# antoinedesbois/Ray-Tracer-Rust

Hardware: AMD Instinct MI355X
Metric: Mrays/sec + frame ms, big_bunny.obj @ 1920x1080 (higher is better)
Workload: dtype f32

## Files before the change

### ray-tracer-rust_amd/csrc/rtx_api.cpp

```cpp
#include <hip/hip_runtime.h>

#include <algorithm>
#include <chrono>
#include <cmath>
#include <cstddef>
#include <cstdio>
#include <cstdlib>
#include <cstring>
#include <initializer_list>
#include <map>
#include <memory>
#include <mutex>
#include <new>
#include <vector>

#include "../../include/rtx.h"
#include "rtx_aim.h"
#include "rtx_device.h"
#include "rtx_light.h"
#include "rtx_query.h"
#include "rtx_shade.h"
#include "rtx_view.h"
#include "scene_prep.h"

// ... 67 lines not shown
    template <class T>
    T *as() const { return static_cast<T *>(static_cast<void *>(mem_)); }
private:
    Owned<void *, Free> mem_;
    size_t cap_ = 0;
};
using DeviceBuffer = GrowOnly<alloc_device, hipFree>;
using PinnedBuffer = GrowOnly<alloc_pinned, hipHostFree>;

struct Sized { DeviceBuffer &buffer; size_t bytes; };
int reserve_all(std::initializer_list<Sized> list)
{
    for (const Sized &s : list) {
        const int rc = s.buffer.reserve(s.bytes);
        if (rc != RTX_OK) return rc;
    }
    return RTX_OK;
}

class DeviceState {
public:
    explicit DeviceState(int dev) : device(dev) {}
    const int device;
    bool uploaded = false;
    size_t last_tiles = 0;
    unsigned long long launches = 0;
    Stream stream;
    Event ev0, ev1;
    Event ring[RTX_TIMING_RING][3];
    Event q_sorted;
    DeviceBuffer nodes, primary_nodes, ref_nodes, tris, shade, samples, lights, light_tour, thr, planes, light_boxes;
    DeviceBuffer d_out, d_counters;
    DeviceBuffer d_redo;
    PinnedBuffer h_stage;
    struct { DeviceBuffer hits, pix_slot, tiles, chunks, results, acc, ctr, buckets, cut; } ws;
    DeviceBuffer q_first, q_second, q_out;
    struct { DeviceBuffer keys, keys_sorted, index, index_sorted, temp; } q_sort;
    struct {
        DeviceBuffer nodes, links;
        float eye[3] = {0.0f, 0.0f, 0.0f};
        hipStream_t on = nullptr;
        bool valid = false;
    } aimed;
    struct {
        DeviceBuffer points;
        Event used;
    } lit;
private:
    ~DeviceState() = default;
    friend struct ReleaseOnDevice;
};

struct ReleaseOnDevice {
    void operator()(DeviceState *st) const
    {
        DeviceGuard g(st->device);
        if (g.status() != hipSuccess) return;
        if (st->stream) (void)hipStreamSynchronize(st->stream);
        delete st;
    }
};

struct DeviceSlot {
    std::mutex mu;
    std::unique_ptr<DeviceState, ReleaseOnDevice> st;
};
// ... 190 lines not shown
uint32_t tiles_rows(uint32_t height, uint32_t first_tile, uint32_t tile_stride, uint32_t tile_rows)
{
    if (!tile_rows || !tile_stride) return 0;
    uint64_t rows = 0;
    for (uint64_t t = first_tile; t * tile_rows < height; t += tile_stride) {
        const uint64_t r0 = t * tile_rows;
        rows += (height - r0 < tile_rows) ? (height - r0) : tile_rows;
    }
    return static_cast<uint32_t>(rows);
}

void fill_stats(RtxStats *s, uint64_t primary_rays, uint32_t shadow_rays_per_hit, const unsigned long long *c,
                double kernel_ms, double total_ms)
{
    std::memset(s, 0, sizeof *s);
    s->primary_rays = primary_rays;
    s->primary_hits = c[0];
    s->shadow_rays = c[0] * shadow_rays_per_hit;
    s->rays = s->primary_rays + s->shadow_rays;
    s->box_tests = c[1];
    s->tri_tests = c[2];
    s->wave_node_visits = c[3];
    s->wave_tri_visits = c[4];
    s->redo_tiles = c[5];
    s->kernel_ms = kernel_ms;
    s->total_ms = total_ms;
}

template <class Before>
int render_launch(DeviceState &st, const rtx::DeviceScene &S, const rtx::TileSpec &ts, uint8_t *d_out,
                  unsigned long long *d_counters, unsigned long long *d_wave_prof, hipStream_t stream, Before before)
{
    int rc;
    if ((rc = st.d_redo.reserve(rtx::trace_redo_bytes(S, ts))) != RTX_OK) return rc;
    rtx::StreamWorkspace ws{};
    bool use_ws = false;
    if (!d_wave_prof && (rc = reserve_stream_ws(st, S, ts, &ws, &use_ws)) != RTX_OK) return rc;
    if ((rc = before()) != RTX_OK) return rc;
    const Event *slot = st.ring[st.launches % RTX_TIMING_RING];
    hipEvent_t phases[3] = {slot[0], slot[1], slot[2]};
    RTX_HIP(rtx::launch_trace_shade(S, ts, d_out, st.d_redo.as<uint32_t>(), use_ws ? &ws : nullptr, d_counters, d_wave_prof,
                                    kernel_variant(), stream, d_wave_prof ? nullptr : phases));
    if (!d_wave_prof && ts.local_rows) ++st.launches;
    return RTX_OK;
}

int launch_on(RtxScene *scene, DeviceSlot &slot, const rtx::TileSpec &ts, bool count)
{
    int rc = ensure_uploaded(scene, slot);
    if (rc != RTX_OK) return rc;
    DeviceState &st = *slot.st;
    const size_t bytes = static_cast<size_t>(ts.local_rows) * scene->prep.width * 3u;
    if ((rc = st.d_out.reserve(bytes ? bytes : 16)) != RTX_OK) return rc;
    unsigned long long *counters = count ? st.d_counters.as<unsigned long long>() : nullptr;
    rc = render_launch(st, device_scene(scene, st), ts, st.d_out.as<uint8_t>(), counters, nullptr, st.stream, [&]() -> int {
        if (count) RTX_HIP(hipMemsetAsync(counters, 0, rtx::kNumCounters * sizeof(unsigned long long), st.stream));
        RTX_HIP(hipEventRecord(st.ev0, st.stream));
        return RTX_OK;
    });
    if (rc != RTX_OK) return rc;
    RTX_HIP(hipEventRecord(st.ev1, st.stream));
    return RTX_OK;
}


rtxq::KeyBox query_key_box(const rtx::PreparedScene &p)
{
    rtxq::KeyBox box{};
    if (p.nodes.empty()) return box;
    const rtx::NodeRec &root = p.nodes[(p.n_global != 0u && p.nodes.size() > 2u) ? 2u : 0u];
    for (int a = 0; a < 3; ++a) {
        const float extent = root.bmax[a] - root.bmin[a];
        const float scale = static_cast<float>(1u << rtxq::kMortonBitsPerAxis) / extent;
        box.lo[a] = root.bmin[a];
        box.scale[a] = (extent > 0.0f && scale > 0.0f && scale < 0x1p100f) ? scale : 0.0f;
// ... 950 lines not shown
```

### ray-tracer-rust_amd/csrc/rtx_device.h

```cpp
#pragma once

#include <hip/hip_runtime.h>

#include <cstdint>

#include "scene_prep.h"

namespace rtx {

struct DeviceScene {
    const NodeRec  *nodes;
    const NodeRec  *primary_nodes;
    const float    *light_tour;
    const NodeRec  *ref_nodes;
    const TriRec   *tris;
    const ShadeRec *shade;
    const TriRec   *planes;
    const float2   *samples;
    const float    *light_points;
    const float    *gamma_thr;
    const float    *light_boxes;
    uint32_t n_nodes, n_ref_nodes, n_samples, n_wide;
    uint32_t width, height;
    uint32_t nb_ray, nb_light;
// ... 46 lines not shown
    uint32_t *buckets;
    CutEntry *cut;
};
constexpr uint32_t kCutInnerFlag = 1u << 29, kCutEndMask = (1u << 26) - 1u;
constexpr uint32_t kCutStreamRecords = kMaxCut + 1u;
__host__ __device__ inline size_t cut_stream_offset(size_t tiles)
{
    return (tiles * kMaxCut * sizeof(CutEntry) + 63u) & ~static_cast<size_t>(63u);
}
struct StreamWorkspaceBytes { size_t hits, pix_slot, tiles, chunks, results, acc, ctr, buckets, cut; };
static_assert(kMaxCut >= 1u && kMaxCut <= 51u && kCutWords * kMaxCut <= 512u, "RTX_MAX_CUT: 1 .. 51 (one staged word per work-item of 512)");
constexpr uint32_t kTileCutShift = 8u;
constexpr uint32_t kTileCompactHits = 8u;
constexpr uint32_t kTileChunk0Kept = 4u;
StreamWorkspaceBytes stream_workspace_bytes(const DeviceScene &S, const TileSpec &ts, uint32_t variant);
constexpr uint32_t kCostBuckets = 64u;
constexpr uint32_t kStreamCtrWords = 4u;

constexpr int kNumCounters = 8;

#ifndef RTX_LIGHT_TOUR
#define RTX_LIGHT_TOUR 1
#endif
static_assert(RTX_LIGHT_TOUR >= 0 && RTX_LIGHT_TOUR <= 2, "RTX_LIGHT_TOUR: 0, 1 or 2");

constexpr uint32_t kVariantStream = 8u;
constexpr uint32_t kVariantPacked = 16u;
constexpr uint32_t kVariantProbe = 32u;
constexpr uint32_t kVariantMask = 63u;
constexpr uint32_t kDefaultVariant = kVariantProbe | 1u;

constexpr size_t kWaveProfWords = 8;
uint32_t trace_tiles_x(const DeviceScene &S, uint32_t variant);
constexpr uint32_t kQueueRedoCount = 0u, kQueueNextTile = 1u, kQueueHeader = 4u;
size_t trace_redo_bytes(const DeviceScene &S, const TileSpec &ts);
hipError_t launch_trace_shade(const DeviceScene &S, const TileSpec &ts, uint8_t *d_out, uint32_t *d_redo,
                              const StreamWorkspace *ws, unsigned long long *d_counters,
                              unsigned long long *d_wave_prof, uint32_t variant, hipStream_t stream,
                              hipEvent_t *phase_events = nullptr);

}
```

### ray-tracer-rust_amd/csrc/rtx_kernel.hip

```cpp
#include <cstdlib>
#include "rtx_traverse.hpp"

namespace rtx {

namespace {

constexpr uint32_t kHitStride = 12u;
__device__ __forceinline__ uint32_t compact_hit_word(uint32_t record, uint32_t word)
{
    return word < 3u ? record * 3u + word : (word < 9u ? 192u + word - 3u : kNone);
}

#ifndef RTX_WAVES_PER_SIMD
#define RTX_WAVES_PER_SIMD 6
#endif
#ifndef RTX_PACKED_WAVES_PER_SIMD
#define RTX_PACKED_WAVES_PER_SIMD 4
#endif

__device__ __forceinline__ uint32_t quantise(const float *__restrict__ thr, float x)
{
    uint32_t b = 0;
#pragma unroll
    for (uint32_t step = 128; step; step >>= 1)
// ... 369 lines not shown
        }
        if (pass && leaf) {
            if (kCutEntriesUsed) out[n_out + (uint32_t)__popcll(m_leaf & below)] = CutEntry{my, my + 1u, nd};
            l_entries[n_out + (uint32_t)__popcll(m_leaf & below)] = CutEntry{my, my + 1u, nd};
            out_stream[n_out + (uint32_t)__popcll(m_leaf & below)] = nd;
            around(nd);
            w += 1u + 3u * nd.link;
        }
        n_out += n_leaf;
        if (n_exp == 0u) break;
        if (pass && !leaf) {
            const uint32_t k = (uint32_t)__popcll(m_exp & below);
            l_front[2u * k] = my + 1u;
            l_front[2u * k + 1u] = nd.info;
        }
        __builtin_amdgcn_fence(__ATOMIC_RELEASE, "wavefront");
        __builtin_amdgcn_wave_barrier();
        n_front = 2u * n_exp;
        my = l_front[lane];
        __builtin_amdgcn_fence(__ATOMIC_ACQUIRE, "wavefront");
        __builtin_amdgcn_wave_barrier();
    }
    weight = wave_sum(w);
    if (n_out >= 2u) {
        NodeDev all;
        all.lox = wave_min(ulx); all.loy = wave_min(uly); all.loz = wave_min(ulz);
        all.hix = wave_max(uhx); all.hiy = wave_max(uhy); all.hiz = wave_max(uhz);
        all.link = 0u; all.info = 0u;
        if (lane == 0) out_stream[kMaxCut] = all;
    }
    return n_out;
}

template <bool COUNT, bool FAST, bool SPHERES, bool WHOLE>
__global__ void __launch_bounds__(64 * kProbeWaves, RTX_PROBE_WAVES_PER_SIMD) probe_kernel(DeviceScene S, TileSpec ts, uint32_t tiles_x, uint32_t n_tiles,
                                                   uint32_t r, StreamWorkspace W, uint8_t *__restrict__ out,
                                                   uint32_t *__restrict__ queue, unsigned long long *__restrict__ counters)
{
    const NodeRec RTX_CONSTANT *nodes = (const NodeRec RTX_CONSTANT *)S.nodes;
    const TriRec RTX_CONSTANT *tris = (const TriRec RTX_CONSTANT *)S.tris;
    __shared__ uint32_t l_front_all[kProbeWaves][128];
    __shared__ CutEntry l_entries_all[kProbeWaves][kMaxCut];
#if RTX_ABLATION
    __shared__ __align__(16) uint32_t l_j1_block[kProbeWaves][kJ1BlockWords];
#endif
    const uint32_t lane = threadIdx.x & 63u;
    const uint32_t wave_in_group = __builtin_amdgcn_readfirstlane(threadIdx.x >> 6);
    uint32_t *const l_front = l_front_all[wave_in_group];
    static_assert(kProbeWaves == 1u, "the XCD mapping assumes one tile per workgroup");
    const uint32_t k = blockIdx.x >> 3;
    const uint32_t tile_id = ((((k >> 6) << 3) + (blockIdx.x & 7u)) << 6) + (k & 63u);
    if (tile_id >= n_tiles) return;
    uint32_t px, py, ly, tile_x, tile_y;
    tile_xy(tile_id, tiles_x, true, tile_x, tile_y);
    const bool in_frame = tile_pixel(S, ts, tile_x, tile_y, lane, px, py, ly);
    WaveCounters wc;
    float dx, dy, dz;
    primary_ray(S, in_frame, px, py, r, dx, dy, dz);
    LaneRay pr = make_ray(in_frame, S.eye[0], S.eye[1], S.eye[2], dx, dy, dz);
#if RTX_EXPERIMENT_PROBE_PHASES
    const unsigned long long pp_t0 = wall_clock64();
#endif
#if RTX_ABLATION
    const bool ok = (S.j1_mode == 2u || S.j1_mode == 3u)
        ? j1_closest_hit_blocks<COUNT>(S.j1_mode, S.tris, S.shade, S.n_prims, pr, wc, lane, l_j1_block[wave_in_group])
        : closest_hit<COUNT, FAST, SPHERES>((const NodeRec RTX_CONSTANT *)S.primary_nodes, tris, S.shade, S.n_nodes, pr, wc, S.n_global);
// ... 88 lines not shown
            (void)length_and_direction(vx, vy, vz, dist_light, sx, sy, sz);
            LaneRay sr = make_ray(hit, hx, hy, hz, sx, sy, sz);
            sr.limit = dist_light;
            WaveCounters probe;
            const bool walked = any_hit<true, FAST, SPHERES>(nodes, tris, S.shade, S.n_nodes, sr, probe, S.n_global);
            weight = (uint32_t)(probe.node_visits + probe.tri_visits);
            if (walked && n_hit == 64u && (flags & 1u)) {
                const unsigned long long occluded = ballot(sr.best_idx != kNone);
                if (lane == 0) {
                    uint32_t *kept = reinterpret_cast<uint32_t *>(W.cut + (size_t)tile_id * kMaxCut);
                    kept[0] = (uint32_t)occluded;
                    kept[1] = (uint32_t)(occluded >> 32);
                }
                flags |= kTileChunk0Kept;
            }
        }
        cost = (unsigned long long)(kChunkFixedCost + weight) * n_chunks;
        if (!(flags & 1u) && n_cut != 0u) cost *= 2u;
    }
    const bool sky = n_hit == 0u && !(flags & 2u);
    if (sky) {
        const size_t pix = (size_t)tile_id * 64u + lane;
        if (r + 1u == S.nb_ray) {
            float a0 = 0.0f, a1 = 0.0f, a2 = 0.0f;
            if (r != 0u) { a0 = W.acc[3u * pix]; a1 = W.acc[3u * pix + 1u]; a2 = W.acc[3u * pix + 2u]; }
            if (in_frame) store_pixel(S, out, px, ly, a0, a1, a2);
        } else if (r == 0u) {
            W.acc[3u * pix] = 0.0f; W.acc[3u * pix + 1u] = 0.0f; W.acc[3u * pix + 2u] = 0.0f;
        }
    }
    if (lane == 0) {
        const bool count_it = !(flags & 2u);
        const uint32_t key = (sky || (flags & 2u)) ? kNone : cost_class(cost);
#if RTX_EXPERIMENT_PROBE_PHASES
        const unsigned long long pp_t2 = wall_clock64();
        const uint32_t walk_ticks = (uint32_t)(pp_t1 - pp_t0) > 0xFFFFu ? 0xFFFFu : (uint32_t)(pp_t1 - pp_t0);
        const uint32_t rest_ticks = (uint32_t)(pp_t2 - pp_t1) > 0xFFFFu ? 0xFFFFu : (uint32_t)(pp_t2 - pp_t1);
        W.tiles[tile_id] = TileDesc{key, n_hit, flags | (n_cut << kTileCutShift), walk_ticks | (rest_ticks << 16)};
#elif RTX_EXPERIMENT_TIMELINE || RTX_EXPERIMENT_PHASES
        W.tiles[tile_id] = TileDesc{key, n_hit, flags | (n_cut << kTileCutShift), 0u};
#else
        W.tiles[tile_id] = TileDesc{key, n_hit, flags | (n_cut << kTileCutShift), counted + (count_it ? n_hit : 0u)};
#endif
        if (COUNT) {
            flush_counters<COUNT>(counters, count_it ? (unsigned long long)n_hit : 0ull, wc);
            if (counters) {
                atomicAdd(&counters[6], wc.node_visits);
                atomicAdd(&counters[7], wc.tri_visits);
            }
        }
    }
}

constexpr uint32_t kOrderHist = kCostBuckets, kOrderCursor = 2u * kCostBuckets, kOrderList = 3u * kCostBuckets;
#ifndef RTX_CLAIM_RUN_LOG
#define RTX_CLAIM_RUN_LOG 10
#endif
constexpr uint32_t kOrderClaim = 8u, kClaimRunLog = RTX_CLAIM_RUN_LOG;
#ifndef RTX_JOB_PRIORITY
#define RTX_JOB_PRIORITY 1
#endif
constexpr bool kJobLevels = RTX_JOB_PRIORITY != 0;
[[maybe_unused]] constexpr float kRaisedShare = 0.25f;
[[maybe_unused]] constexpr uint32_t kOrderRaisedEnd = 1u;
[[maybe_unused]] constexpr uint32_t kJobLevelRaised = 2u;
__device__ __forceinline__ uint32_t claimed_index(uint32_t group, uint32_t k)
{
    return ((((k >> kClaimRunLog) << 3) + group) << kClaimRunLog) + (k & ((1u << kClaimRunLog) - 1u));
}
__device__ __forceinline__ uint32_t claim_job(uint32_t *__restrict__ buckets, uint32_t n_jobs, uint32_t group0, uint32_t &groups_done,
                                              uint32_t *pos = nullptr)
{
    while (groups_done < 8u) {
        const uint32_t g = (group0 + groups_done) & 7u;
        const uint32_t idx = claimed_index(g, atomicAdd(&buckets[kOrderClaim + g], 1u));
        if (pos) *pos = idx;
        if (idx < n_jobs) return buckets[kOrderList + idx];
        ++groups_done;
    }
    return kNone;
}
constexpr float kSplitScaleMin = 0.25f;
#ifndef RTX_TILE_PARTS_MAX
#define RTX_TILE_PARTS_MAX 4
#endif
constexpr uint32_t kMaxTileParts = RTX_TILE_PARTS_MAX;
static_assert(kMaxTileParts >= 1u && kMaxTileParts <= 16u && (kMaxTileParts & (kMaxTileParts - 1u)) == 0u, "parts: a power of two <= 16");
constexpr uint32_t kNotMine = 0xFFFFFFFEu;
constexpr uint32_t kJobTileBits = 25u, kJobTileMask = (1u << kJobTileBits) - 1u, kJobPartsShift = 28u, kJobCompactShift = 30u;
static_assert(kMaxTileParts <= 8u, "a job word holds three bits of part number and two of log2(parts)");
__device__ __forceinline__ float class_cost(uint32_t k)
{
    if (k == 0u) return 0.0f;
    const uint32_t lz = (k - 1u) >> 1, half = (k - 1u) & 1u;
    return lz ? (float)(2u + half) * (float)(1u << (lz - 1u)) : 1.0f;
}

__global__ void __launch_bounds__(256) reset_kernel(uint32_t *__restrict__ queue, uint32_t first, uint32_t end,
                                                    uint32_t *__restrict__ buckets, uint32_t n)
{
    for (uint32_t i = first + threadIdx.x; i < end; i += 256u) queue[i] = 0u;
    for (uint32_t i = threadIdx.x; i < n; i += 256u) buckets[i] = 0u;
}

__global__ void __launch_bounds__(1024) count_classes_kernel(uint32_t n_tiles, StreamWorkspace W)
{
    __shared__ uint32_t count[kCostBuckets];
    const uint32_t tid = threadIdx.x, lane = tid & 63u;
    if (tid < kCostBuckets) count[tid] = 0u;
    __syncthreads();
    const uint32_t i = blockIdx.x * 1024u + tid;
    const uint32_t key = i < n_tiles ? W.tiles[i].first : kNone;
    unsigned long long todo = ballot(key != kNone);
    while (todo != 0ull) {
        const uint32_t k0 = __builtin_amdgcn_readfirstlane(__shfl(key, __ffsll((long long)todo) - 1));
        const unsigned long long same = ballot(key == k0);
        if (lane == (uint32_t)(__ffsll((long long)same) - 1)) atomicAdd(&count[k0], (uint32_t)__popcll(same));
        todo &= ~same;
    }
    __syncthreads();
    if (tid < kCostBuckets && count[tid] != 0u) atomicAdd(&W.buckets[kOrderHist + tid], count[tid]);
}

__global__ void __launch_bounds__(1024) order_tiles_kernel(uint32_t n_tiles, StreamWorkspace W, uint32_t shade_grid, float split_share)
{
    __shared__ uint32_t count[kCostBuckets], start[kCostBuckets], parts_log[kCostBuckets], jobs[kCostBuckets];
    __shared__ float weight[kCostBuckets];
#if RTX_JOB_PRIORITY
    __shared__ float raised_cost;
#endif
    const uint32_t tid = threadIdx.x, lane = tid & 63u;
    if (tid < kCostBuckets) {
        count[tid] = 0u;
        weight[tid] = (float)W.buckets[kOrderHist + tid] * class_cost(tid);
    }
    __syncthreads();
    const uint32_t i = blockIdx.x * 1024u + tid;
    const uint32_t key = i < n_tiles ? W.tiles[i].first : kNone;
    uint32_t slot = 0u;
    unsigned long long todo = ballot(key != kNone);
    while (todo != 0ull) {
        const uint32_t k0 = __builtin_amdgcn_readfirstlane(__shfl(key, __ffsll((long long)todo) - 1));
        const unsigned long long same = ballot(key == k0);
        uint32_t off = 0u;
        if (lane == (uint32_t)(__ffsll((long long)same) - 1)) off = atomicAdd(&count[k0], (uint32_t)__popcll(same));
        off = __shfl(off, __ffsll((long long)same) - 1);
        if (key == k0) slot = off + (uint32_t)__popcll(same & ((1ull << lane) - 1ull));
        todo &= ~same;
    }
    if (tid < kCostBuckets) {
        float total = 0.0f;
        uint32_t scheduled = 0u;
        for (uint32_t k = 0; k < kCostBuckets; ++k) { total += weight[k]; scheduled += W.buckets[kOrderHist + k]; }
        const float per_wg = (float)scheduled / (float)shade_grid;
        const float scale = per_wg >= 16.0f ? 1.0f : (per_wg <= 16.0f * kSplitScaleMin ? kSplitScaleMin : per_wg * (1.0f / 16.0f));
        const float limit = split_share * scale * total / (float)shade_grid;
        const uint32_t most_parts = per_wg < 3.0f ? kMaxTileParts : (kMaxTileParts < 4u ? kMaxTileParts : 4u);
        uint32_t lg = 0u;
        while ((1u << lg) < most_parts && class_cost(tid) > limit * (float)(1u << lg)) ++lg;
        parts_log[tid] = lg;
        jobs[tid] = W.buckets[kOrderHist + tid] << lg;
#if RTX_JOB_PRIORITY
        if (tid == 0) raised_cost = limit * kRaisedShare;
#endif
    }
    __syncthreads();
    if (tid < kCostBuckets) {
        uint32_t before = 0u;
        for (uint32_t k = tid + 1u; k < kCostBuckets; ++k) before += jobs[k];
        const uint32_t mine = count[tid];
        start[tid] = before + ((mine ? atomicAdd(&W.buckets[kOrderCursor + tid], mine) : 0u) << parts_log[tid]);
        if (blockIdx.x == 0 && tid == 0) W.buckets[0] = before + jobs[0];
#if RTX_JOB_PRIORITY
        const bool raised = tid != 0u && class_cost(tid) >= raised_cost;
        const bool cheaper_raised = tid > 1u && class_cost(tid - 1u) >= raised_cost;
        if (blockIdx.x == 0 && raised && !cheaper_raised) W.buckets[kOrderRaisedEnd] = before + jobs[tid];
#endif
    }
    __syncthreads();
    if (key != kNone) {
        const uint32_t lg = parts_log[key];
        uint32_t *dst = W.buckets + kOrderList + start[key] + (slot << lg);
        const uint32_t form = (W.tiles[i].flags & kTileCompactHits) ? 1u << kJobCompactShift : 0u;
        for (uint32_t p = 0; p < (1u << lg); ++p) dst[p] = i | (p << kJobTileBits) | (lg << kJobPartsShift) | form;
    }
}

#ifndef RTX_SHADE_WAVES_PER_SIMD
#define RTX_SHADE_WAVES_PER_SIMD 8
#endif

#ifndef RTX_SHADE_CUT_WAVES_PER_SIMD
#define RTX_SHADE_CUT_WAVES_PER_SIMD 8
#endif
constexpr int kShadePriority = 1;
[[maybe_unused]] constexpr uint32_t kCtlJobLevel = 12u;
__device__ __forceinline__ void set_wave_priority(uint32_t level)
{
    switch (level) {
    case 0u: __builtin_amdgcn_s_setprio(0); break;
    case 1u: __builtin_amdgcn_s_setprio(1); break;
    case 2u: __builtin_amdgcn_s_setprio(2); break;
    default: __builtin_amdgcn_s_setprio(3); break;
    }
}
template <bool COUNT, bool FAST, int NW, bool SPHERES, bool WHOLE>
__global__ void __launch_bounds__(64 * NW, COUNT ? 1 : (WHOLE ? RTX_SHADE_WAVES_PER_SIMD : RTX_SHADE_CUT_WAVES_PER_SIMD))
shade_tiles_kernel(DeviceScene S, TileSpec ts, uint32_t batch, uint32_t tiles_x, uint32_t n_tiles, uint32_t r,
                   StreamWorkspace W, uint8_t *__restrict__ out, uint32_t *__restrict__ queue,
// ... 17 lines not shown
    const NodeRec RTX_CONSTANT *nodes = (const NodeRec RTX_CONSTANT *)S.nodes;
    const TriRec RTX_CONSTANT *tris = (const TriRec RTX_CONSTANT *)S.tris;
    const TriRec RTX_CONSTANT *planes = (const TriRec RTX_CONSTANT *)S.planes;
    const bool have_plane = planes != nullptr;
    TriRec plane0 = {};
    if (have_plane) {
        plane0.v0[0] = planes->v0[0]; plane0.v0[1] = planes->v0[1]; plane0.v0[2] = planes->v0[2];
        plane0.e1[0] = planes->e1[0]; plane0.e1[1] = planes->e1[1]; plane0.e1[2] = planes->e1[2];
        plane0.e2[0] = planes->e2[0]; plane0.e2[1] = planes->e2[1]; plane0.e2[2] = planes->e2[2];
        plane0.bmin[0] = planes->bmin[0];
    }
    const uint32_t lane = threadIdx.x & 63u;
    const uint32_t wave = __builtin_amdgcn_readfirstlane(threadIdx.x >> 6);
    WaveCounters wc;
    const float denom = (float)(S.nb_ray * S.nb_light);
    const DenomDiv denom_d = denom_div(denom);
    static_assert(sizeof(HitRec) == kHitStride * sizeof(float), "the LDS hit record is the HBM hit record");

#if RTX_EXPERIMENT_TIMELINE
    uint32_t tl_tile = kNone;
    unsigned long long tl_t0 = 0;
#endif
    const uint32_t n_jobs = W.buckets[0];
    uint32_t job_ahead = kNone, q_ahead = 0u;
#if RTX_JOB_PRIORITY
    static_assert(NW + 4 <= (int)kCtlJobLevel && kCtlJobLevel < kCtlWords, "the level's word lies behind the run counters");
    const uint32_t raised_end = W.buckets[kOrderRaisedEnd];
#endif
    [[maybe_unused]] uint32_t pos_ahead = 0u;
    bool have_ahead = false;
    constexpr bool xcd_queues = WHOLE;
    const uint32_t group0 = blockIdx.x & 7u;
    uint32_t groups_done = 0u, g_ahead = 0u;
    const bool lights_once = S.nb_light <= batch;
    if (lights_once)
        for (uint32_t k = threadIdx.x; k < kLightStride * S.nb_light; k += 64u * NW) l_light[k] = S.light_tour[kLightStride * (r * S.nb_light) + k];
    for (;;) {
        if (threadIdx.x == 0) {
            if (!have_ahead) {
                if (xcd_queues) {
                    job_ahead = claim_job(W.buckets, n_jobs, group0, groups_done, kJobLevels ? &pos_ahead : nullptr);
                } else {
                    const uint32_t q = atomicAdd(&queue[kQueueNextTile], 1u);
                    job_ahead = q < n_jobs ? W.buckets[kOrderList + q] : kNone;
                    if (kJobLevels) pos_ahead = q;
                }
            }
            l_ctl[3] = job_ahead;
#if RTX_JOB_PRIORITY
            l_ctl[kCtlJobLevel] = pos_ahead < raised_end ? kJobLevelRaised : 0u;
#endif
            have_ahead = false;
            l_ctl[1] = 0u;
#if RTX_EXPERIMENT_TIMELINE
            const unsigned long long now = wall_clock64();
            if (tl_tile != kNone) atomicAdd(&W.tiles[tl_tile].pad, (uint32_t)(now - tl_t0));
            tl_tile = l_ctl[3] == kNone ? kNone : (l_ctl[3] & kJobTileMask);
            tl_t0 = now;
#endif
        }
        __syncthreads();
        const uint32_t job = __builtin_amdgcn_readfirstlane(l_ctl[3]);
        if (job == kNone) break;
        __builtin_amdgcn_s_setprio(kShadePriority);
#if RTX_EXPERIMENT_PHASES
        unsigned long long ph_t[6] = {(unsigned long long)wall_clock64(), 0, 0, 0, 0, 0};
// ... 295 lines not shown
#if RTX_EXPERIMENT_PHASES
        ph_t[5] = wall_clock64();
        if (threadIdx.x == 0 && n_cut == 0u && n_hit != 0u && !skip) {
            for (int k = 0; k < 5; ++k) atomicAdd(&W.tiles[k].pad, (uint32_t)(ph_t[k + 1] - ph_t[k]));
            atomicAdd(&W.tiles[5].pad, 1u);
        }
#endif
    }
    if (COUNT && lane == 0) flush_counters<COUNT>(counters, 0ull, wc);
}

namespace {

#ifndef RTX_SPLIT_SHARE_PERCENT
#define RTX_SPLIT_SHARE_PERCENT 100
#endif
constexpr float kSplitShare = RTX_SPLIT_SHARE_PERCENT * 0.01f;
float split_share()
{
#if RTX_ABLATION
    static const float v = [] {
        const char *e = getenv("RTX_SPLIT_SHARE");
        const float x = e ? strtof(e, nullptr) : 0.0f;
        return x > 0.0f ? x : kSplitShare;
    }();
    return v;
#else
    return kSplitShare;
#endif
}

template <bool COUNT, bool FAST, bool SPHERES>
hipError_t launch_probe(const DeviceScene &S, const TileSpec &ts, uint8_t *d_out, uint32_t *d_redo,
                        const StreamWorkspace &W, unsigned long long *d_counters, hipStream_t stream, hipEvent_t *ev)
{
#ifndef RTX_SHADE_NW
#define RTX_SHADE_NW 8
#endif
    constexpr int NW = RTX_SHADE_NW;
    const bool whole = S.n_nodes > S.cut_max_nodes;
    const uint32_t batch = S.nb_light < kMaxLightBatch ? (S.nb_light ? S.nb_light : 1u) : kMaxLightBatch;
#if RTX_ABLATION
    const size_t lds_bytes = (static_cast<size_t>(lds_floats(batch)) + (S.j1_mode == 1u ? kJ1WindowWords : 0u)) * sizeof(float);
#else
    const size_t lds_bytes = static_cast<size_t>(lds_floats(batch)) * sizeof(float);
#endif
    const uint32_t tiles_x = (S.width + 7u) / 8u, tiles_y = (ts.local_rows + 7u) / 8u;
    const uint32_t n_tiles = numbered_tiles(tiles_x, tiles_y);
    static thread_local int cached_dev = -1, cached_blocks = 0;
    static thread_local size_t cached_lds = 0;
    static thread_local bool cached_whole = false;
    int dev = 0;
    hipError_t e = hipGetDevice(&dev);
    if (e != hipSuccess) return e;
    if (dev != cached_dev || lds_bytes != cached_lds || whole != cached_whole) {
        int per_cu = 0, cus = 0;
        e = whole ? hipOccupancyMaxActiveBlocksPerMultiprocessor(&per_cu, shade_tiles_kernel<COUNT, FAST, NW, SPHERES, true>, 64 * NW, lds_bytes)
                  : hipOccupancyMaxActiveBlocksPerMultiprocessor(&per_cu, shade_tiles_kernel<COUNT, FAST, NW, SPHERES, false>, 64 * NW, lds_bytes);
        if (e != hipSuccess) return e;
        if ((e = hipDeviceGetAttribute(&cus, hipDeviceAttributeMultiprocessorCount, dev)) != hipSuccess) return e;
        cached_blocks = (per_cu > 0 ? per_cu : 1) * (cus > 0 ? cus : 1);
        cached_dev = dev;
        cached_lds = lds_bytes;
        cached_whole = whole;
    }
    if (n_tiles > kJobTileMask) return hipErrorInvalidValue;
    const uint64_t most_jobs = (uint64_t)n_tiles * kMaxTileParts;
    const uint32_t grid = most_jobs < static_cast<uint64_t>(cached_blocks) ? (uint32_t)most_jobs : static_cast<uint32_t>(cached_blocks);
    for (uint32_t r = 0; r < S.nb_ray; ++r) {
        hipLaunchKernelGGL(reset_kernel, dim3(1), dim3(256), 0, stream, d_redo, r == 0u ? 0u : kQueueNextTile,
                           r == 0u ? kQueueHeader : kQueueNextTile + 1u, W.buckets, 3u * kCostBuckets);
        hipLaunchKernelGGL(whole ? (probe_kernel<COUNT, FAST, SPHERES, true>) : (probe_kernel<COUNT, FAST, SPHERES, false>),
                           dim3(512u * ((n_tiles + 511u) / 512u)), dim3(64 * kProbeWaves), 0, stream,
                           S, ts, tiles_x, n_tiles, r, W, d_out, d_redo, d_counters);
        hipLaunchKernelGGL(count_classes_kernel, dim3((n_tiles + 1023u) / 1024u), dim3(1024), 0, stream, n_tiles, W);
        hipLaunchKernelGGL(order_tiles_kernel, dim3((n_tiles + 1023u) / 1024u), dim3(1024), 0, stream, n_tiles, W, grid, split_share());
        if (ev && r == 0u && (e = hipEventRecord(ev[1], stream)) != hipSuccess) return e;
        if (whole)
            hipLaunchKernelGGL((shade_tiles_kernel<COUNT, FAST, NW, SPHERES, true>), dim3(grid), dim3(64 * NW), lds_bytes, stream, S, ts,
                               batch, tiles_x, n_tiles, r, W, d_out, d_redo, d_counters);
        else
            hipLaunchKernelGGL((shade_tiles_kernel<COUNT, FAST, NW, SPHERES, false>), dim3(grid), dim3(64 * NW), lds_bytes, stream, S, ts,
                               batch, tiles_x, n_tiles, r, W, d_out, d_redo, d_counters);
        if ((e = hipGetLastError()) != hipSuccess) return e;
    }
    hipLaunchKernelGGL((reference_tiles_kernel<COUNT, SPHERES>), dim3(n_tiles < 1024u ? n_tiles : 1024u), dim3(64), 0, stream,
                       S, ts, tiles_x, d_out, d_redo, d_counters, true);
    return hipGetLastError();
}

}

#if RTX_ABLATION
#include "rtx_ablation_kernels.hpp"
#endif

uint32_t trace_tiles_x(const DeviceScene &S, uint32_t variant) { return (S.width + 7u) / 8u; }

size_t trace_redo_bytes(const DeviceScene &S, const TileSpec &ts)
{
    return sizeof(uint32_t) * (kQueueHeader + static_cast<size_t>(numbered_tiles((S.width + 7u) / 8u, (ts.local_rows + 7u) / 8u)));
}

StreamWorkspaceBytes stream_workspace_bytes(const DeviceScene &S, const TileSpec &ts, uint32_t variant)
{
    const bool two_pass = (variant & kVariantProbe) != 0u;
    const size_t tiles = two_pass ? numbered_tiles((S.width + 7u) / 8u, (ts.local_rows + 7u) / 8u)
                                  : static_cast<size_t>((S.width + 7u) / 8u) * ((ts.local_rows + 7u) / 8u);
    const size_t pixels = tiles * 64u;
    const bool streamed = (variant & kVariantStream) != 0u, probe = (variant & kVariantProbe) != 0u;
    StreamWorkspaceBytes b;
    b.hits = pixels * sizeof(HitRec);
    b.pix_slot = pixels * sizeof(uint32_t);
    b.tiles = tiles * sizeof(TileDesc);
    b.chunks = streamed ? (pixels * S.nb_light / 64u + tiles + 1u) * sizeof(uint2) : 0u;
    b.results = streamed ? pixels * (S.nb_light ? S.nb_light : 1u) * sizeof(float) : 0u;
    b.acc = S.nb_ray > 1u ? pixels * 3u * sizeof(float) : 0u;
    b.ctr = kStreamCtrWords * sizeof(uint32_t);
    b.buckets = probe ? (3u * kCostBuckets + tiles * kMaxTileParts) * sizeof(uint32_t) : 0u;
    b.cut = probe ? cut_stream_offset(tiles) + tiles * kCutStreamRecords * sizeof(NodeDev) : 0u;
    return b;
}

static hipError_t launch_dispatch(const DeviceScene &S, const TileSpec &ts, uint8_t *d_out, uint32_t *d_redo,
                                  const StreamWorkspace *ws, unsigned long long *d_counters,
                                  unsigned long long *d_wave_prof, uint32_t variant, hipStream_t stream, hipEvent_t *ev)
{
#if RTX_ABLATION
    if (!((variant & kVariantProbe) && ws && !d_wave_prof))
        return launch_dispatch_ablation(S, ts, d_out, d_redo, ws, d_counters, d_wave_prof, variant, stream);
    if (!(variant & 1u)) {
        if (S.n_spheres)
            return d_counters ? launch_probe<true, false, true>(S, ts, d_out, d_redo, *ws, d_counters, stream, ev)
                              : launch_probe<false, false, true>(S, ts, d_out, d_redo, *ws, d_counters, stream, ev);
        return d_counters ? launch_probe<true, false, false>(S, ts, d_out, d_redo, *ws, d_counters, stream, ev)
                          : launch_probe<false, false, false>(S, ts, d_out, d_redo, *ws, d_counters, stream, ev);
    }
#else
    if (variant != kDefaultVariant || !ws || d_wave_prof) return hipErrorInvalidValue;
#endif
    if (S.n_spheres)
        return d_counters ? launch_probe<true, true, true>(S, ts, d_out, d_redo, *ws, d_counters, stream, ev)
                          : launch_probe<false, true, true>(S, ts, d_out, d_redo, *ws, d_counters, stream, ev);
    return d_counters ? launch_probe<true, true, false>(S, ts, d_out, d_redo, *ws, d_counters, stream, ev)
                      : launch_probe<false, true, false>(S, ts, d_out, d_redo, *ws, d_counters, stream, ev);
}

hipError_t launch_trace_shade(const DeviceScene &S, const TileSpec &ts, uint8_t *d_out, uint32_t *d_redo,
                              const StreamWorkspace *ws, unsigned long long *d_counters,
                              unsigned long long *d_wave_prof, uint32_t variant, hipStream_t stream,
                              hipEvent_t *phase_events)
{
    if (ts.local_rows == 0) return hipSuccess;
    hipError_t e;
    if (phase_events && (e = hipEventRecord(phase_events[0], stream)) != hipSuccess) return e;
    const bool probe = (variant & kVariantProbe) && ws && !d_wave_prof;
    if (phase_events && !probe && (e = hipEventRecord(phase_events[1], stream)) != hipSuccess) return e;
    e = launch_dispatch(S, ts, d_out, d_redo, ws, d_counters, d_wave_prof, variant, stream, probe ? phase_events : nullptr);
    if (e != hipSuccess) return e;
    if (phase_events && (e = hipEventRecord(phase_events[2], stream)) != hipSuccess) return e;
    return hipSuccess;
}

}

#ifndef RTX_EXPERIMENT_TIMELINE
#define RTX_EXPERIMENT_TIMELINE 0
#endif
#ifndef RTX_EXPERIMENT_PHASES
#define RTX_EXPERIMENT_PHASES 0
#endif
#ifndef RTX_EXPERIMENT_PROBE_PHASES
#define RTX_EXPERIMENT_PROBE_PHASES 0
#endif
#ifndef RTX_ABLATION
#define RTX_ABLATION 0
#endif
#define RTX_SW_STR2(x) #x
#define RTX_SW_STR(x) RTX_SW_STR2(x)
#define RTX_SW(x) " " #x "=" RTX_SW_STR(x)
extern "C" __attribute__((used, visibility("hidden"))) const char rtx_build_switches_text[] = "rtx-build-switches:"
    RTX_SW(RTX_CLAIM_RUN_LOG) RTX_SW(RTX_CUT_DRAW_MIN) RTX_SW(RTX_CUT_UNION_MIN) RTX_SW(RTX_LIGHT_BATCH) RTX_SW(RTX_LIGHT_TOUR) RTX_SW(RTX_MAX_CUT)
    RTX_SW(RTX_PACKED_WAVES_PER_SIMD) RTX_SW(RTX_PROBE_VISIT_SCALE) RTX_SW(RTX_PROBE_WAVES_PER_SIMD)
    RTX_SW(RTX_SHADE_CUT_WAVES_PER_SIMD) RTX_SW(RTX_SHADE_NW) RTX_SW(RTX_SHADE_WAVES_PER_SIMD)
    RTX_SW(RTX_SPLIT_SHARE_PERCENT) RTX_SW(RTX_TILE_PARTS_MAX) RTX_SW(RTX_WAVES_PER_SIMD) RTX_SW(RTX_JOB_PRIORITY)
    RTX_SW(RTX_EXPERIMENT_TIMELINE) RTX_SW(RTX_EXPERIMENT_PHASES) RTX_SW(RTX_EXPERIMENT_PROBE_PHASES) RTX_SW(RTX_ABLATION);
#undef RTX_SW
```

Before: 136,900.

## Drop per-pass reset and class-count kernels via double-buffered histogram sets

Removes the per-pass reset_kernel launch and, in the non-whole path, the count_classes_kernel. The probe kernel now builds a sharded cost-class histogram with atomics directly. Histogram and cursor state is double-buffered across passes, and the queue words across launches, so order_tiles_kernel can zero the next set and reset the claim words itself. The shade kernel prefetches its first job from blockIdx and the raised-priority share shrinks for small job counts. This cuts kernel launches and serial tiny kernels per frame, at the cost of extra atomics in the probe kernel and a more intricate host-side state machine that must re-zero the buffers when they are reallocated.

```diff
diff --git a/ray-tracer-rust_amd/csrc/rtx_api.cpp b/ray-tracer-rust_amd/csrc/rtx_api.cpp
--- a/ray-tracer-rust_amd/csrc/rtx_api.cpp
+++ b/ray-tracer-rust_amd/csrc/rtx_api.cpp
@@ -123,6 +123,8 @@
     DeviceBuffer nodes, primary_nodes, ref_nodes, tris, shade, samples, lights, light_tour, thr, planes, light_boxes;
     DeviceBuffer d_out, d_counters;
     DeviceBuffer d_redo;
+    bool launch_words_ready = false;
+    uint32_t words_launches = 0, words_passes = 0;
     PinnedBuffer h_stage;
     struct { DeviceBuffer hits, pix_slot, tiles, chunks, results, acc, ctr, buckets, cut; } ws;
     DeviceBuffer q_first, q_second, q_out;
@@ -379,6 +381,7 @@
                   unsigned long long *d_counters, unsigned long long *d_wave_prof, hipStream_t stream, Before before)
 {
     int rc;
+    const size_t redo_cap = st.d_redo.capacity(), buckets_cap = st.ws.buckets.capacity();
     if ((rc = st.d_redo.reserve(rtx::trace_redo_bytes(S, ts))) != RTX_OK) return rc;
     rtx::StreamWorkspace ws{};
     bool use_ws = false;
@@ -386,8 +389,19 @@
     if ((rc = before()) != RTX_OK) return rc;
     const Event *slot = st.ring[st.launches % RTX_TIMING_RING];
     hipEvent_t phases[3] = {slot[0], slot[1], slot[2]};
+    const bool two_pass = use_ws && (kernel_variant() & rtx::kVariantProbe) != 0u && ts.local_rows != 0u;
+    if (two_pass && (!st.launch_words_ready || st.d_redo.capacity() != redo_cap || st.ws.buckets.capacity() != buckets_cap)) {
+        RTX_HIP(rtx::zero_launch_words(st.d_redo.as<uint32_t>(), ws, stream));
+        st.words_launches = st.words_passes = 0;
+    }
+    if (ts.local_rows) st.launch_words_ready = false;
     RTX_HIP(rtx::launch_trace_shade(S, ts, d_out, st.d_redo.as<uint32_t>(), use_ws ? &ws : nullptr, d_counters, d_wave_prof,
-                                    kernel_variant(), stream, d_wave_prof ? nullptr : phases));
+                                    kernel_variant(), stream, d_wave_prof ? nullptr : phases, st.words_launches, st.words_passes));
+    if (two_pass) {
+        st.launch_words_ready = true;
+        ++st.words_launches;
+        st.words_passes += S.nb_ray;
+    }
     if (!d_wave_prof && ts.local_rows) ++st.launches;
     return RTX_OK;
 }
diff --git a/ray-tracer-rust_amd/csrc/rtx_device.h b/ray-tracer-rust_amd/csrc/rtx_device.h
--- a/ray-tracer-rust_amd/csrc/rtx_device.h
+++ b/ray-tracer-rust_amd/csrc/rtx_device.h
@@ -102,11 +102,12 @@
 
 constexpr size_t kWaveProfWords = 8;
 uint32_t trace_tiles_x(const DeviceScene &S, uint32_t variant);
-constexpr uint32_t kQueueRedoCount = 0u, kQueueNextTile = 1u, kQueueHeader = 4u;
+constexpr uint32_t kQueueRedoCount = 0u, kQueueNextTile = 1u, kQueueHeader = 4u, kQueueSlotStride = 2u;
 size_t trace_redo_bytes(const DeviceScene &S, const TileSpec &ts);
 hipError_t launch_trace_shade(const DeviceScene &S, const TileSpec &ts, uint8_t *d_out, uint32_t *d_redo,
                               const StreamWorkspace *ws, unsigned long long *d_counters,
                               unsigned long long *d_wave_prof, uint32_t variant, hipStream_t stream,
-                              hipEvent_t *phase_events = nullptr);
+                              hipEvent_t *phase_events = nullptr, uint32_t launch_no = 0u, uint32_t pass_no = 0u);
+hipError_t zero_launch_words(uint32_t *d_redo, const StreamWorkspace &ws, hipStream_t stream);
 
 }
diff --git a/ray-tracer-rust_amd/csrc/rtx_kernel.hip b/ray-tracer-rust_amd/csrc/rtx_kernel.hip
--- a/ray-tracer-rust_amd/csrc/rtx_kernel.hip
+++ b/ray-tracer-rust_amd/csrc/rtx_kernel.hip
@@ -425,6 +425,16 @@
     return n_out;
 }
 
+constexpr uint32_t kHistShardsLog = 8u, kHistShards = 1u << kHistShardsLog;
+constexpr uint32_t kOrderHist = kCostBuckets;
+constexpr uint32_t kOrderCursor = kHistShards * kCostBuckets;
+constexpr uint32_t kOrderSetWords = kOrderCursor + kCostBuckets;
+__host__ __device__ inline StreamWorkspace counting_set(StreamWorkspace W, uint32_t set)
+{
+    W.buckets += set * kOrderSetWords;
+    return W;
+}
+
 template <bool COUNT, bool FAST, bool SPHERES, bool WHOLE>
 __global__ void __launch_bounds__(64 * kProbeWaves, RTX_PROBE_WAVES_PER_SIMD) probe_kernel(DeviceScene S, TileSpec ts, uint32_t tiles_x, uint32_t n_tiles,
                                                    uint32_t r, StreamWorkspace W, uint8_t *__restrict__ out,
@@ -579,6 +589,7 @@
     if (lane == 0) {
         const bool count_it = !(flags & 2u);
         const uint32_t key = (sky || (flags & 2u)) ? kNone : cost_class(cost);
+        if (!WHOLE && key != kNone) atomicAdd(&W.buckets[kOrderHist + (tile_id & (kHistShards - 1u)) * kCostBuckets + key], 1u);
 #if RTX_EXPERIMENT_PROBE_PHASES
         const unsigned long long pp_t2 = wall_clock64();
         const uint32_t walk_ticks = (uint32_t)(pp_t1 - pp_t0) > 0xFFFFu ? 0xFFFFu : (uint32_t)(pp_t1 - pp_t0);
@@ -599,7 +610,7 @@
     }
 }
 
-constexpr uint32_t kOrderHist = kCostBuckets, kOrderCursor = 2u * kCostBuckets, kOrderList = 3u * kCostBuckets;
+constexpr uint32_t kOrderList = kOrderHist + 2u * kOrderSetWords;
 #ifndef RTX_CLAIM_RUN_LOG
 #define RTX_CLAIM_RUN_LOG 10
 #endif
@@ -608,7 +619,7 @@
 #define RTX_JOB_PRIORITY 1
 #endif
 constexpr bool kJobLevels = RTX_JOB_PRIORITY != 0;
-[[maybe_unused]] constexpr float kRaisedShare = 0.25f;
+[[maybe_unused]] constexpr float kRaisedShare = 0.25f, kRaisedShareSmall = 0.125f, kRaisedSmallJobs = 64.0f;
 [[maybe_unused]] constexpr uint32_t kOrderRaisedEnd = 1u;
 [[maybe_unused]] constexpr uint32_t kJobLevelRaised = 2u;
 __device__ __forceinline__ uint32_t claimed_index(uint32_t group, uint32_t k)
@@ -669,19 +680,32 @@
     if (tid < kCostBuckets && count[tid] != 0u) atomicAdd(&W.buckets[kOrderHist + tid], count[tid]);
 }
 
-__global__ void __launch_bounds__(1024) order_tiles_kernel(uint32_t n_tiles, StreamWorkspace W, uint32_t shade_grid, float split_share)
-{
-    __shared__ uint32_t count[kCostBuckets], start[kCostBuckets], parts_log[kCostBuckets], jobs[kCostBuckets];
-    __shared__ float weight[kCostBuckets];
+__global__ void __launch_bounds__(1024) order_tiles_kernel(uint32_t n_tiles, StreamWorkspace W, uint32_t shade_grid, float split_share,
+                                                           uint32_t hist_set, uint32_t first_claim, uint32_t *__restrict__ queue,
+                                                           uint32_t *__restrict__ next_redo_count)
+{
+    __shared__ uint32_t count[kCostBuckets], start[kCostBuckets], parts_log[kCostBuckets], jobs[kCostBuckets], hist[kCostBuckets];
 #if RTX_JOB_PRIORITY
     __shared__ float raised_cost;
 #endif
     const uint32_t tid = threadIdx.x, lane = tid & 63u;
+    uint32_t *const set = counting_set(W, hist_set).buckets + kOrderHist;
+    uint32_t *const next_set = counting_set(W, hist_set ^ 1u).buckets + kOrderHist;
     if (tid < kCostBuckets) {
         count[tid] = 0u;
-        weight[tid] = (float)W.buckets[kOrderHist + tid] * class_cost(tid);
-    }
+        hist[tid] = 0u;
+    }
+    static_assert(kHistShards % 16u == 0u && kCostBuckets == 64u, "1024 work-items: 16 shards x 64 classes at a time");
+    uint32_t in_shards = 0u;
+    for (uint32_t s = tid >> 6; s < kHistShards; s += 16u) in_shards += set[s * kCostBuckets + lane];
     __syncthreads();
+    if (in_shards != 0u) atomicAdd(&hist[lane], in_shards);
+    for (uint32_t w = blockIdx.x * 1024u + tid; w < kOrderSetWords; w += gridDim.x * 1024u) next_set[w] = 0u;
+    if (blockIdx.x == 0) {
+        if (tid < 8u) W.buckets[kOrderClaim + tid] = 0u;
+        if (tid == 8u) queue[kQueueNextTile] = first_claim;
+        if (tid == 9u) *next_redo_count = 0u;
+    }
     const uint32_t i = blockIdx.x * 1024u + tid;
     const uint32_t key = i < n_tiles ? W.tiles[i].first : kNone;
     uint32_t slot = 0u;
@@ -695,10 +719,11 @@
         if (key == k0) slot = off + (uint32_t)__popcll(same & ((1ull << lane) - 1ull));
         todo &= ~same;
     }
+    __syncthreads();
     if (tid < kCostBuckets) {
         float total = 0.0f;
         uint32_t scheduled = 0u;
-        for (uint32_t k = 0; k < kCostBuckets; ++k) { total += weight[k]; scheduled += W.buckets[kOrderHist + k]; }
+        for (uint32_t k = 0; k < kCostBuckets; ++k) { total += (float)hist[k] * class_cost(k); scheduled += hist[k]; }
         const float per_wg = (float)scheduled / (float)shade_grid;
         const float scale = per_wg >= 16.0f ? 1.0f : (per_wg <= 16.0f * kSplitScaleMin ? kSplitScaleMin : per_wg * (1.0f / 16.0f));
         const float limit = split_share * scale * total / (float)shade_grid;
@@ -706,9 +731,9 @@
         uint32_t lg = 0u;
         while ((1u << lg) < most_parts && class_cost(tid) > limit * (float)(1u << lg)) ++lg;
         parts_log[tid] = lg;
-        jobs[tid] = W.buckets[kOrderHist + tid] << lg;
+        jobs[tid] = hist[tid] << lg;
 #if RTX_JOB_PRIORITY
-        if (tid == 0) raised_cost = limit * kRaisedShare;
+        if (tid == 0) raised_cost = limit * (per_wg < kRaisedSmallJobs ? kRaisedShareSmall : kRaisedShare);
 #endif
     }
     __syncthreads();
@@ -716,12 +741,13 @@
         uint32_t before = 0u;
         for (uint32_t k = tid + 1u; k < kCostBuckets; ++k) before += jobs[k];
         const uint32_t mine = count[tid];
-        start[tid] = before + ((mine ? atomicAdd(&W.buckets[kOrderCursor + tid], mine) : 0u) << parts_log[tid]);
+        start[tid] = before + ((mine ? atomicAdd(&set[kOrderCursor + tid], mine) : 0u) << parts_log[tid]);
         if (blockIdx.x == 0 && tid == 0) W.buckets[0] = before + jobs[0];
 #if RTX_JOB_PRIORITY
         const bool raised = tid != 0u && class_cost(tid) >= raised_cost;
         const bool cheaper_raised = tid > 1u && class_cost(tid - 1u) >= raised_cost;
         if (blockIdx.x == 0 && raised && !cheaper_raised) W.buckets[kOrderRaisedEnd] = before + jobs[tid];
+        if (blockIdx.x == 0 && tid == kCostBuckets - 1u && !raised) W.buckets[kOrderRaisedEnd] = 0u;
 #endif
     }
     __syncthreads();
@@ -805,6 +831,11 @@
     constexpr bool xcd_queues = WHOLE;
     const uint32_t group0 = blockIdx.x & 7u;
     uint32_t groups_done = 0u, g_ahead = 0u;
+    if (!xcd_queues) {
+        job_ahead = blockIdx.x < n_jobs ? W.buckets[kOrderList + blockIdx.x] : kNone;
+        if (kJobLevels) pos_ahead = blockIdx.x;
+        have_ahead = true;
+    }
     const bool lights_once = S.nb_light <= batch;
     if (lights_once)
         for (uint32_t k = threadIdx.x; k < kLightStride * S.nb_light; k += 64u * NW) l_light[k] = S.light_tour[kLightStride * (r * S.nb_light) + k];
@@ -1166,7 +1197,8 @@
 
 template <bool COUNT, bool FAST, bool SPHERES>
 hipError_t launch_probe(const DeviceScene &S, const TileSpec &ts, uint8_t *d_out, uint32_t *d_redo,
-                        const StreamWorkspace &W, unsigned long long *d_counters, hipStream_t stream, hipEvent_t *ev)
+                        const StreamWorkspace &W, unsigned long long *d_counters, hipStream_t stream, hipEvent_t *ev,
+                        uint32_t launch_no, uint32_t pass_no)
 {
 #ifndef RTX_SHADE_NW
 #define RTX_SHADE_NW 8
@@ -1201,25 +1233,28 @@
     if (n_tiles > kJobTileMask) return hipErrorInvalidValue;
     const uint64_t most_jobs = (uint64_t)n_tiles * kMaxTileParts;
     const uint32_t grid = most_jobs < static_cast<uint64_t>(cached_blocks) ? (uint32_t)most_jobs : static_cast<uint32_t>(cached_blocks);
+    uint32_t *const queue = d_redo + (launch_no & 1u) * kQueueSlotStride;
+    uint32_t *const next_redo_count = d_redo + ((launch_no + 1u) & 1u) * kQueueSlotStride + kQueueRedoCount;
     for (uint32_t r = 0; r < S.nb_ray; ++r) {
-        hipLaunchKernelGGL(reset_kernel, dim3(1), dim3(256), 0, stream, d_redo, r == 0u ? 0u : kQueueNextTile,
-                           r == 0u ? kQueueHeader : kQueueNextTile + 1u, W.buckets, 3u * kCostBuckets);
+        const uint32_t hist_set = (pass_no + r) & 1u;
+        const StreamWorkspace Wp = counting_set(W, hist_set);
         hipLaunchKernelGGL(whole ? (probe_kernel<COUNT, FAST, SPHERES, true>) : (probe_kernel<COUNT, FAST, SPHERES, false>),
                            dim3(512u * ((n_tiles + 511u) / 512u)), dim3(64 * kProbeWaves), 0, stream,
-                           S, ts, tiles_x, n_tiles, r, W, d_out, d_redo, d_counters);
-        hipLaunchKernelGGL(count_classes_kernel, dim3((n_tiles + 1023u) / 1024u), dim3(1024), 0, stream, n_tiles, W);
-        hipLaunchKernelGGL(order_tiles_kernel, dim3((n_tiles + 1023u) / 1024u), dim3(1024), 0, stream, n_tiles, W, grid, split_share());
+                           S, ts, tiles_x, n_tiles, r, Wp, d_out, queue, d_counters);
+        if (whole) hipLaunchKernelGGL(count_classes_kernel, dim3((n_tiles + 1023u) / 1024u), dim3(1024), 0, stream, n_tiles, Wp);
+        hipLaunchKernelGGL(order_tiles_kernel, dim3((n_tiles + 1023u) / 1024u), dim3(1024), 0, stream, n_tiles, W, grid, split_share(),
+                           hist_set, whole ? 0u : grid, queue, next_redo_count);
         if (ev && r == 0u && (e = hipEventRecord(ev[1], stream)) != hipSuccess) return e;
         if (whole)
             hipLaunchKernelGGL((shade_tiles_kernel<COUNT, FAST, NW, SPHERES, true>), dim3(grid), dim3(64 * NW), lds_bytes, stream, S, ts,
-                               batch, tiles_x, n_tiles, r, W, d_out, d_redo, d_counters);
+                               batch, tiles_x, n_tiles, r, W, d_out, queue, d_counters);
         else
             hipLaunchKernelGGL((shade_tiles_kernel<COUNT, FAST, NW, SPHERES, false>), dim3(grid), dim3(64 * NW), lds_bytes, stream, S, ts,
-                               batch, tiles_x, n_tiles, r, W, d_out, d_redo, d_counters);
+                               batch, tiles_x, n_tiles, r, W, d_out, queue, d_counters);
         if ((e = hipGetLastError()) != hipSuccess) return e;
     }
     hipLaunchKernelGGL((reference_tiles_kernel<COUNT, SPHERES>), dim3(n_tiles < 1024u ? n_tiles : 1024u), dim3(64), 0, stream,
-                       S, ts, tiles_x, d_out, d_redo, d_counters, true);
+                       S, ts, tiles_x, d_out, queue, d_counters, true);
     return hipGetLastError();
 }
 
@@ -1231,9 +1266,15 @@
 
 uint32_t trace_tiles_x(const DeviceScene &S, uint32_t variant) { return (S.width + 7u) / 8u; }
 
+hipError_t zero_launch_words(uint32_t *d_redo, const StreamWorkspace &W, hipStream_t stream)
+{
+    hipLaunchKernelGGL(reset_kernel, dim3(1), dim3(256), 0, stream, d_redo, 0u, kQueueSlotStride + kQueueHeader, W.buckets, kOrderList);
+    return hipGetLastError();
+}
+
 size_t trace_redo_bytes(const DeviceScene &S, const TileSpec &ts)
 {
-    return sizeof(uint32_t) * (kQueueHeader + static_cast<size_t>(numbered_tiles((S.width + 7u) / 8u, (ts.local_rows + 7u) / 8u)));
+    return sizeof(uint32_t) * (kQueueSlotStride + kQueueHeader + static_cast<size_t>(numbered_tiles((S.width + 7u) / 8u, (ts.local_rows + 7u) / 8u)));
 }
 
 StreamWorkspaceBytes stream_workspace_bytes(const DeviceScene &S, const TileSpec &ts, uint32_t variant)
@@ -1251,46 +1292,47 @@
     b.results = streamed ? pixels * (S.nb_light ? S.nb_light : 1u) * sizeof(float) : 0u;
     b.acc = S.nb_ray > 1u ? pixels * 3u * sizeof(float) : 0u;
     b.ctr = kStreamCtrWords * sizeof(uint32_t);
-    b.buckets = probe ? (3u * kCostBuckets + tiles * kMaxTileParts) * sizeof(uint32_t) : 0u;
+    b.buckets = probe ? (kOrderList + tiles * kMaxTileParts) * sizeof(uint32_t) : 0u;
     b.cut = probe ? cut_stream_offset(tiles) + tiles * kCutStreamRecords * sizeof(NodeDev) : 0u;
     return b;
 }
 
 static hipError_t launch_dispatch(const DeviceScene &S, const TileSpec &ts, uint8_t *d_out, uint32_t *d_redo,
                                   const StreamWorkspace *ws, unsigned long long *d_counters,
-                                  unsigned long long *d_wave_prof, uint32_t variant, hipStream_t stream, hipEvent_t *ev)
+                                  unsigned long long *d_wave_prof, uint32_t variant, hipStream_t stream, hipEvent_t *ev,
+                                  uint32_t launch_no, uint32_t pass_no)
 {
 #if RTX_ABLATION
     if (!((variant & kVariantProbe) && ws && !d_wave_prof))
         return launch_dispatch_ablation(S, ts, d_out, d_redo, ws, d_counters, d_wave_prof, variant, stream);
     if (!(variant & 1u)) {
         if (S.n_spheres)
-            return d_counters ? launch_probe<true, false, true>(S, ts, d_out, d_redo, *ws, d_counters, stream, ev)
-                              : launch_probe<false, false, true>(S, ts, d_out, d_redo, *ws, d_counters, stream, ev);
-        return d_counters ? launch_probe<true, false, false>(S, ts, d_out, d_redo, *ws, d_counters, stream, ev)
-                          : launch_probe<false, false, false>(S, ts, d_out, d_redo, *ws, d_counters, stream, ev);
+            return d_counters ? launch_probe<true, false, true>(S, ts, d_out, d_redo, *ws, d_counters, stream, ev, launch_no, pass_no)
+                              : launch_probe<false, false, true>(S, ts, d_out, d_redo, *ws, d_counters, stream, ev, launch_no, pass_no);
+        return d_counters ? launch_probe<true, false, false>(S, ts, d_out, d_redo, *ws, d_counters, stream, ev, launch_no, pass_no)
+                          : launch_probe<false, false, false>(S, ts, d_out, d_redo, *ws, d_counters, stream, ev, launch_no, pass_no);
     }
 #else
     if (variant != kDefaultVariant || !ws || d_wave_prof) return hipErrorInvalidValue;
 #endif
     if (S.n_spheres)
-        return d_counters ? launch_probe<true, true, true>(S, ts, d_out, d_redo, *ws, d_counters, stream, ev)
-                          : launch_probe<false, true, true>(S, ts, d_out, d_redo, *ws, d_counters, stream, ev);
-    return d_counters ? launch_probe<true, true, false>(S, ts, d_out, d_redo, *ws, d_counters, stream, ev)
-                      : launch_probe<false, true, false>(S, ts, d_out, d_redo, *ws, d_counters, stream, ev);
+        return d_counters ? launch_probe<true, true, true>(S, ts, d_out, d_redo, *ws, d_counters, stream, ev, launch_no, pass_no)
+                          : launch_probe<false, true, true>(S, ts, d_out, d_redo, *ws, d_counters, stream, ev, launch_no, pass_no);
+    return d_counters ? launch_probe<true, true, false>(S, ts, d_out, d_redo, *ws, d_counters, stream, ev, launch_no, pass_no)
+                      : launch_probe<false, true, false>(S, ts, d_out, d_redo, *ws, d_counters, stream, ev, launch_no, pass_no);
 }
 
 hipError_t launch_trace_shade(const DeviceScene &S, const TileSpec &ts, uint8_t *d_out, uint32_t *d_redo,
                               const StreamWorkspace *ws, unsigned long long *d_counters,
                               unsigned long long *d_wave_prof, uint32_t variant, hipStream_t stream,
-                              hipEvent_t *phase_events)
+                              hipEvent_t *phase_events, uint32_t launch_no, uint32_t pass_no)
 {
     if (ts.local_rows == 0) return hipSuccess;
     hipError_t e;
     if (phase_events && (e = hipEventRecord(phase_events[0], stream)) != hipSuccess) return e;
     const bool probe = (variant & kVariantProbe) && ws && !d_wave_prof;
     if (phase_events && !probe && (e = hipEventRecord(phase_events[1], stream)) != hipSuccess) return e;
-    e = launch_dispatch(S, ts, d_out, d_redo, ws, d_counters, d_wave_prof, variant, stream, probe ? phase_events : nullptr);
+    e = launch_dispatch(S, ts, d_out, d_redo, ws, d_counters, d_wave_prof, variant, stream, probe ? phase_events : nullptr, launch_no, pass_no);
     if (e != hipSuccess) return e;
     if (phase_events && (e = hipEventRecord(phase_events[2], stream)) != hipSuccess) return e;
     return hipSuccess;
```

Measured after the change: 140,500 (median of 6 runs). 2.6% higher.
